# Julian-Wyatt/AnoDDPM

Measured on AMD Instinct MI355X. Metric: reverse-diffusion images/sec @256x256 T=1000 simplex, higher is better.
Workload: dtype f32; 1 GPU; 256x256 simplex(8 oct) T=1000 base128 attn16,8 batch4/GPU (BASELINE config 2); per_gpu_batch=4, global_batch=4, T=1000, parallelism=batch-sharded x1 (no data-path collective), output_finite=True

## Files before the change

anoddpm_amd/csrc/pointwise.hip:

```cpp
#include "common.h"

namespace {

typedef float f32x4 __attribute__((ext_vector_type(4)));
typedef float f32x16 __attribute__((ext_vector_type(16)));

constexpr int PW_WAVES = 8;
constexpr int PW_NT = PW_WAVES * 64;

template <int NB, int KMAX, int DBG = 0>
__global__ __launch_bounds__(PW_NT) void pointwise_stream_kernel(const anoddpm_igemm_args a, const int tiles, const int tiles_per_image)
{
    constexpr int NBP = NB + 2;
    constexpr int NTN = NB / 32;
    __shared__ __attribute__((aligned(16))) f32x4 wl[(KMAX / 4) * NBP];
    const int tid = threadIdx.x, lane = tid & 63, wave = tid >> 6;
    const int p = lane & 31, h = lane >> 5;
    const int K = a.c0 + a.c1, N = a.N;
    const int n0 = blockIdx.y * NB;
    const int nchunks = K >> 5;

    {
        const f32x4 *__restrict__ wg = reinterpret_cast<const f32x4 *>(a.bmat);
        const int total = (K >> 2) * NB;
        for (int idx = tid; idx < total; idx += PW_NT) {
            const int q = idx / NB, n = idx - q * NB;
            wl[q * NBP + n] = wg[(int64_t)q * N + n0 + n];
        }
    }
    __syncthreads();

    const int gw = blockIdx.x * PW_WAVES + wave, stride = gridDim.x * PW_WAVES;
    if (gw >= tiles) return;
    const int my_tiles = (tiles - gw + stride - 1) / stride;

    f32x4 ring[4][4];
    int ld_tile = 0, ld_chunk = 0;
    const float *ld_base0 = nullptr, *ld_base1 = nullptr;
    auto set_tile = [&](int t) {
        const int tile = gw + (t < my_tiles ? t : my_tiles - 1) * stride;
        const int b = tile / tiles_per_image, pl = (tile - b * tiles_per_image) * 32 + p;
        ld_base0 = a.a0 + (int64_t)b * a.a0_bs + (int64_t)pl * a.a0_ld + h * 16;
        ld_base1 = a.c1 ? a.a1 + (int64_t)b * a.a1_bs + (int64_t)pl * a.a1_ld + h * 16 : ld_base0;
    };
    auto issue = [&](f32x4 (&dst)[4]) {
        if ((DBG & 2) && ld_tile + ld_chunk > 2) return;
        const int c = ld_chunk * 32;
        const float *src = c < a.c0 ? ld_base0 + c : ld_base1 + (c - a.c0);
#pragma unroll
        for (int i = 0; i < 4; ++i) dst[i] = *reinterpret_cast<const f32x4 *>(src + 4 * i);
        if (++ld_chunk == nchunks) { ld_chunk = 0; set_tile(++ld_tile); }
    };
    set_tile(0);
    issue(ring[0]);
    issue(ring[1]);
    issue(ring[2]);
    if (wave >= PW_WAVES / 2 && my_tiles >= 2 && !(DBG & 4)) {
        for (int i = 0; i < nchunks / 2; ++i) __builtin_amdgcn_s_sleep(127);
    }

    const f32x4 *wrow = wl + h * 4 * NBP + p;
    f32x4 bq[2][NTN];
#pragma unroll
    for (int nt = 0; nt < NTN; ++nt) bq[0][nt] = wrow[nt * 32];
    for (int t = 0; t < my_tiles; ++t) {
        f32x16 acc[NTN];
#pragma unroll
        for (int nt = 0; nt < NTN; ++nt)
#pragma unroll
            for (int r = 0; r < 16; ++r) acc[nt][r] = 0.f;
        for (int j0 = 0; j0 < nchunks; j0 += 4) {
#pragma unroll
            for (int s = 0; s < 4; ++s) {
                issue(ring[(s + 3) & 3]);
                const int j = j0 + s;
                const f32x4 *wq = wrow + j * 8 * NBP;
                const f32x4 *wn = wrow + (j + 1 == nchunks ? 0 : j + 1) * 8 * NBP;
#pragma unroll
                for (int i = 0; i < 4; ++i) {
                    const f32x4 *nx = i < 3 ? wq + (i + 1) * NBP : wn;
#pragma unroll
                    for (int nt = 0; nt < NTN; ++nt) bq[(i + 1) & 1][nt] = nx[nt * 32];
                    __builtin_amdgcn_sched_barrier(0);
#pragma unroll
                    for (int e = 0; e < 4; ++e)
#pragma unroll
                        for (int nt = 0; nt < NTN; ++nt)
                            acc[nt] = __builtin_amdgcn_mfma_f32_32x32x2f32(bq[i & 1][nt][e], ring[s][i][e], acc[nt], 0, 0, 0);
                    __builtin_amdgcn_sched_barrier(0);
                }
            }
        }
        const int tile = gw + t * stride;
        const int b = tile / tiles_per_image, pl = (tile - b * tiles_per_image) * 32 + p;
        float *__restrict__ O = a.out + (int64_t)b * a.o_bs + (int64_t)pl * a.out_ld + n0 + 4 * h;
        const float *R = a.res ? a.res + (int64_t)b * a.r_bs + (int64_t)pl * a.res_ld + n0 + 4 * h : nullptr;
        const float *TE = a.temb ? a.temb + (int64_t)b * a.temb_ld + n0 + 4 * h : nullptr;
        const float *BI = a.bias ? a.bias + n0 + 4 * h : nullptr;
#pragma unroll
        for (int nt = 0; nt < NTN; ++nt) {
            f32x4 rv[4], add[4];
#pragma unroll
            for (int g = 0; g < 4; ++g) {
                const int c = nt * 32 + g * 8;
                rv[g] = R ? *reinterpret_cast<const f32x4 *>(R + c) : f32x4{0.f, 0.f, 0.f, 0.f};
                add[g] = BI ? *reinterpret_cast<const f32x4 *>(BI + c) : f32x4{0.f, 0.f, 0.f, 0.f};
                if (TE) add[g] += *reinterpret_cast<const f32x4 *>(TE + c);
            }
#pragma unroll
            for (int g = 0; g < 4; ++g) {
                f32x4 v;
#pragma unroll
                for (int e = 0; e < 4; ++e) v[e] = a.alpha * acc[nt][g * 4 + e] + add[g][e] + rv[g][e];
                if (!(DBG & 1) || v[0] == 12345.678f) *reinterpret_cast<f32x4 *>(O + nt * 32 + g * 8) = v;
            }
        }
    }
}

}

namespace anoddpm {

int launch_pointwise_stream(const anoddpm_igemm_args *a, hipStream_t s)
{
    const int K = a->c0 + a->c1;
    const int64_t P = (int64_t)a->H * a->W;
    ANODDPM_REQUIRE(a->ks == 1 && a->a_mode == 0 && a->b_mode == 0 && a->heads == 1 && a->ksplit == 1,
                    "pointwise stream: needs an unsplit 1x1 convolution with packed weights");
    ANODDPM_REQUIRE(!a->gn_scale && a->act == 0 && !a->stats, "pointwise stream: no fused GroupNorm / activation / statistics");
    ANODDPM_REQUIRE(K % 128 == 0 && a->c0 % 32 == 0 && K <= 512, "pointwise stream: K must be a multiple of 128, <= 512, sources split at a multiple of 32");
    ANODDPM_REQUIRE(P % 32 == 0 && a->N % 64 == 0, "pointwise stream: H*W must be a multiple of 32 and N of 64");
    const int64_t tiles = a->B * (P / 32);
    ANODDPM_REQUIRE(tiles < ((int64_t)1 << 31), "pointwise stream: too many pixels");
    const bool wide = (a->N % 128 == 0) && K <= 256;
    const int NB = wide ? 128 : 64;
    const int ny = a->N / NB;
    int gx = 256 / ny;
    const int64_t need = (tiles + PW_WAVES - 1) / PW_WAVES;
    if (gx > need) gx = (int)need;
    if (gx < 1) gx = 1;
    const dim3 grid((unsigned)gx, (unsigned)ny);
#ifdef ANODDPM_ABLATE
    const int dbg = anoddpm::g_debug[3];
#endif
    const int tpi = (int)(P / 32);
#define PW_LAUNCH(NB_, KMAX_, DBG_) \
    hipLaunchKernelGGL((pointwise_stream_kernel<NB_, KMAX_, DBG_>), grid, dim3(PW_NT), 0, s, *a, (int)tiles, tpi)
#ifdef ANODDPM_ABLATE
    if (wide && dbg == 1) PW_LAUNCH(128, 256, 1);
    else if (wide && dbg == 2) PW_LAUNCH(128, 256, 2);
    else if (wide && dbg == 3) PW_LAUNCH(128, 256, 3);
    else if (wide && dbg == 4) PW_LAUNCH(128, 256, 4);
    else
#endif
    if (wide) PW_LAUNCH(128, 256, 0);
    else PW_LAUNCH(64, 512, 0);
#undef PW_LAUNCH
    return check_launch("igemm(pointwise stream)");
}

}
```

anoddpm_amd/csrc/smallmap.hip:

```cpp
#include "common.h"

using anoddpm::silu_f;

namespace {

typedef float f32x4 __attribute__((ext_vector_type(4)));

constexpr int SM_NT = 512;

__host__ __device__ constexpr int sm_kch(int ks) { return ks == 3 ? 256 : 512; }
__host__ __device__ constexpr int sm_hpix(int ks, int tm, int w) { return ks == 1 ? tm : (tm / w + 2) * (w + 2); }

__device__ __forceinline__ __amdgpu_buffer_rsrc_t sm_rsrc(const float *base)
{
    return __builtin_amdgcn_make_buffer_rsrc(const_cast<float *>(base), 0, 0x7ffffffe, 0x00020000);
}
__device__ __forceinline__ f32x4 sm_bld4(__amdgpu_buffer_rsrc_t r, unsigned lane_bytes, unsigned wave_bytes)
{
    return __builtin_bit_cast(f32x4, __builtin_amdgcn_raw_buffer_load_b128(r, (int)lane_bytes, (int)wave_bytes, 0));
}

template <int KS, int RT, int CT, int LOG2W>
__global__ __launch_bounds__(SM_NT) void smallmap_kernel(const anoddpm_igemm_args a)
{
// ... 127 lines not shown
                    for (int u = 0; u < 4; ++u)
                        if (r0 + u < rows) { s += (double)v[u].x; qq += (double)v[u].y; }
                }
            }
            csum[2 * c] = s; csum[2 * c + 1] = qq;
        }
        __syncthreads();
        if (tid < groups) {
            double S = 0.0, Q = 0.0;
            for (int c = tid * cpg; c < (tid + 1) * cpg; ++c) { S += csum[2 * c]; Q += csum[2 * c + 1]; }
            const double n = (double)P * cpg;
            const double mean = S / n;
            double var = Q / n - mean * mean;
            var = var > 0.0 ? var : 0.0;
            gst[2 * tid] = mean;
            gst[2 * tid + 1] = 1.0 / sqrt(var + (double)a.fold_eps);
        }
        __syncthreads();
        for (int c = tid; c < Kpad; c += SM_NT) {
            float scv = 0.f, shv = 0.f;
            if (c < K) {
                const int g = c / cpg;
                const double sc = gst[2 * g + 1] * (double)a.fold_gamma[c];
                scv = (float)sc;
                shv = (float)((double)a.fold_beta[c] - gst[2 * g] * sc);
            }
            aff_sc[c] = scv; aff_sh[c] = shv;
        }
        __syncthreads();
    } else if (a.gn_scale) {
        for (int c = tid; c < Kpad; c += SM_NT) {
            aff_sc[c] = c < K ? a.gn_scale[(int64_t)b * a.gn_ld + c] : 0.f;
            aff_sh[c] = c < K ? a.gn_shift[(int64_t)b * a.gn_ld + c] : 0.f;
        }
        __syncthreads();
    }
    store_A(0);
    __syncthreads();

    int hp0[RT];
#pragma unroll
    for (int rt = 0; rt < RT; ++rt) {
        const int m = rt * 16 + l16;
        hp0[rt] = (KS == 1 ? m : (m >> LOG2W) * HP + (m & (W - 1))) * PITCH + 4 * q;
    }
    f32x4 acc[RT][CT];
#pragma unroll
    for (int rt = 0; rt < RT; ++rt)
#pragma unroll
        for (int ct = 0; ct < CT; ++ct) acc[rt][ct] = f32x4{0.f, 0.f, 0.f, 0.f};

    for (int chunk = 0; chunk < nchunks; ++chunk) {
        const float *Ab = Abuf + (chunk & (nbuf - 1)) * (HPIX * PITCH) + wave * CPW;
        const bool more = chunk + 1 < nchunks;
        if (more) load_A(chunk + 1);
        f32x4 av[2][RT];
        auto read_frags = [&](int s, int set) {
            const int tap = s / SPT, i = s % SPT;
            const int toff = (KS == 1 ? 0 : (tap / 3) * HP + (tap % 3)) * PITCH + 16 * i;
#pragma unroll
            for (int rt = 0; rt < RT; ++rt) av[set][rt] = *reinterpret_cast<const f32x4 *>(Ab + hp0[rt] + toff);
        };
        read_frags(0, 0);
#pragma unroll
        for (int s = 0; s < SPC; ++s) {
            const int cur = s & 1, slot = s % PD;
            if (s + 1 < SPC) read_frags(s + 1, cur ^ 1);
#pragma unroll
            for (int e = 0; e < 4; ++e)
#pragma unroll
                for (int rt = 0; rt < RT; ++rt)
#pragma unroll
                    for (int ct = 0; ct < CT; ++ct)
                        acc[rt][ct] = __builtin_amdgcn_mfma_f32_16x16x4f32(av[cur][rt][e], ring[slot][ct][e], acc[rt][ct], 0, 0, 0);
            const unsigned o = (s + PD < SPC) ? b_off(chunk, s + PD) : b_off(chunk + 1, s + PD - SPC);
#pragma unroll
            for (int ct = 0; ct < CT; ++ct) ring[slot][ct] = sm_bld4(rW, ulane, o + ct * 256u);
            __builtin_amdgcn_sched_barrier(0);
        }
        if (more) {
            if (nbuf == 1) __syncthreads();
            store_A(chunk + 1);
        }
        __syncthreads();
    }

    auto red_at = [&](int slot, int rt, int ct, int e) { return red + ((slot * TM + rt * 16 + 4 * q + e) * RP + ct * 16 + l16); };
    if (wave >= 4) {
#pragma unroll
        for (int rt = 0; rt < RT; ++rt)
#pragma unroll
            for (int ct = 0; ct < CT; ++ct)
#pragma unroll
                for (int e = 0; e < 4; ++e) *red_at(wave - 4, rt, ct, e) = acc[rt][ct][e];
    }
    __syncthreads();
    if (wave < 4) {
#pragma unroll
        for (int rt = 0; rt < RT; ++rt)
#pragma unroll
            for (int ct = 0; ct < CT; ++ct)
#pragma unroll
                for (int e = 0; e < 4; ++e) acc[rt][ct][e] += *red_at(wave, rt, ct, e);
    }
    __syncthreads();
    if (wave < 4) {
#pragma unroll
        for (int rt = 0; rt < RT; ++rt)
#pragma unroll
            for (int ct = 0; ct < CT; ++ct)
#pragma unroll
                for (int e = 0; e < 4; ++e) *red_at(wave, rt, ct, e) = acc[rt][ct][e];
    }
    __syncthreads();
    float *O = a.out + (int64_t)b * a.o_bs;
    const float *R = a.res ? a.res + (int64_t)b * a.r_bs : nullptr;
    const float *TE = a.temb ? a.temb + (int64_t)b * a.temb_ld : nullptr;
    constexpr int ITEMS = TM * (TN / 4);
    for (int it = tid; it < ITEMS; it += SM_NT) {
        const int row = it / (TN / 4), c4 = it - row * (TN / 4);
        const float *r0 = red + row * RP + c4 * 4;
        f32x4 v = *reinterpret_cast<const f32x4 *>(r0);
        v += *reinterpret_cast<const f32x4 *>(r0 + TM * RP);
        v += *reinterpret_cast<const f32x4 *>(r0 + 2 * TM * RP);
        v += *reinterpret_cast<const f32x4 *>(r0 + 3 * TM * RP);
        const int n = n0 + c4 * 4;
        v = v * a.alpha;
        if (a.bias) v += *reinterpret_cast<const f32x4 *>(a.bias + n);
        if (TE) v += *reinterpret_cast<const f32x4 *>(TE + n);
        if (R) v += *reinterpret_cast<const f32x4 *>(R + (int64_t)(p0 + row) * a.res_ld + n);
        *reinterpret_cast<f32x4 *>(O + (int64_t)(p0 + row) * a.out_ld + n) = v;
        if (a.stats) *reinterpret_cast<f32x4 *>(red + (4 * TM + row) * RP + c4 * 4) = v;
    }
    if (a.stats) {
        __syncthreads();
        if (tid < TN) {
            const float *col = red + 4 * TM * RP + tid;
            float s = 0.f, qq = 0.f;
#pragma unroll 4
            for (int r = 0; r < TM; ++r) { const float v = col[r * RP]; s += v; qq += v * v; }
            float *st = a.stats + (((int64_t)b * (P / TM) + p0 / TM) * N + n0 + tid) * 2;
            st[0] = s; st[1] = qq;
        }
    }
}

}

namespace anoddpm {

int smallmap_tile(int ks, int H, int W, int K, int c0, int N, int B)
{
    const int P = H * W;
    if (!(ks == 1 || ks == 3) || P > 256 || P < 16 || (W != 4 && W != 8 && W != 16) || H * W != P) return 0;
    if (K % 16 || c0 % 4 || K > 1024 || N % 32 || K < 16) return 0;
    const int M = B * P;
    static const int cand[4][2] = {{2, 6}, {1, 6}, {2, 2}, {1, 2}};
    int best = 0;
    for (int c = 0; c < 4; ++c) {
        const int rt = cand[c][0], ct = cand[c][1];
        const int tm = 16 * rt, tn = 16 * ct;
        if (P % tm || tm % W || N % tn) continue;
        if (ks == 3 && ct == 6) continue;
        const int wgs = (M / tm) * (N / tn);
        if (wgs >= 200) return rt * 16 + ct;
        best = rt * 16 + ct;
    }
    return best;
}

int launch_smallmap(const anoddpm_igemm_args *a, hipStream_t s)
{
    const int K = a->c0 + a->c1;
    ANODDPM_REQUIRE(a->b_mode == 0 && a->heads == 1 && a->a_mode == 0 && a->ksplit == 1, "smallmap: needs packed weights, heads 1, a_mode 0, ksplit 1");
    const int tile = smallmap_tile(a->ks, a->H, a->W, K, a->c0, a->N, a->B);
    ANODDPM_REQUIRE(tile != 0, "smallmap: shape not supported (H*W <= 256, W in {4, 8, 16}, K %% 16 == 0, 16 <= K <= 1024, N %% 32 == 0)");
    ANODDPM_REQUIRE(a->c1 == 0 || a->a1, "smallmap: dual source needs a1");
    ANODDPM_REQUIRE(a->out_ld % 4 == 0 && (!a->res || a->res_ld % 4 == 0) && a->a0_ld % 4 == 0 && (a->c1 == 0 || a->a1_ld % 4 == 0),
                    "smallmap: pixel strides must be multiples of 4 floats");
    ANODDPM_REQUIRE(!a->tail_csum, "smallmap: no split-K tail");
    ANODDPM_REQUIRE(!a->gn_scale || a->gn_shift, "smallmap: gn_scale without gn_shift");
    if (a->fold_gamma) {
        ANODDPM_REQUIRE(a->fold_beta && a->fold_stats0 && (a->c1 == 0 || a->fold_stats1), "smallmap: GroupNorm fold: null pointer");
        ANODDPM_REQUIRE(a->fold_groups >= 1 && a->fold_groups <= 64 && K % a->fold_groups == 0, "smallmap: GroupNorm fold: bad group count");
        ANODDPM_REQUIRE((a->fold_fmt0 != 0 || a->fold_rows0 >= 1) && (a->c1 == 0 || a->fold_fmt1 != 0 || a->fold_rows1 >= 1),
                        "smallmap: GroupNorm fold: statistics rows missing");
    }
    const int rt = tile >> 4, ct = tile & 15;
    const int TM = 16 * rt, TN = 16 * ct;
    const int P = a->H * a->W;
    const int kch = sm_kch(a->ks);
    const int nchunks = (K + kch - 1) / kch, Kpad = nchunks * kch;
    const int hpix = sm_hpix(a->ks, TM, a->W);
    size_t stage = (size_t)(nchunks > 1 ? 2 : 1) * hpix * (kch + 4) * sizeof(float);
    const size_t fold = (size_t)(2 * Kpad + 128) * sizeof(double);
    const size_t redb = (size_t)5 * TM * (TN + 4) * sizeof(float);
    if (stage < fold) stage = fold;
    if (stage < redb) stage = redb;
    const size_t lds = (size_t)2 * Kpad * sizeof(float) + stage;
    ANODDPM_REQUIRE(lds <= 160 * 1024, "smallmap: LDS budget exceeded");
    dim3 grid((unsigned)(a->N / TN), (unsigned)((int64_t)a->B * P / TM));
#define SM_LAUNCH(KS_, RT_, CT_, LW_)                                                                                     \
    do {                                                                                                                  \
        static bool attr_done[ANODDPM_MAX_DEV];                                                                           \
        if (int rc_ = allow_big_lds(reinterpret_cast<const void *>(&smallmap_kernel<KS_, RT_, CT_, LW_>), attr_done,      \
                                    "igemm(smallmap)"))                                                                   \
            return rc_;                                                                                                   \
        hipLaunchKernelGGL((smallmap_kernel<KS_, RT_, CT_, LW_>), grid, dim3(SM_NT), lds, s, *a);                         \
        return check_launch("igemm(smallmap)");                                                                           \
    } while (0)
    const int lw = a->W == 4 ? 2 : (a->W == 8 ? 3 : 4);
    if (a->ks == 3) {
        if (rt == 1 && ct == 2) { if (lw == 2) SM_LAUNCH(3, 1, 2, 2); if (lw == 3) SM_LAUNCH(3, 1, 2, 3); SM_LAUNCH(3, 1, 2, 4); }
        if (rt == 2 && ct == 2) { if (lw == 2) SM_LAUNCH(3, 2, 2, 2); if (lw == 3) SM_LAUNCH(3, 2, 2, 3); SM_LAUNCH(3, 2, 2, 4); }
    } else {
        if (rt == 1 && ct == 2) SM_LAUNCH(1, 1, 2, 3);
        if (rt == 1 && ct == 6) SM_LAUNCH(1, 1, 6, 3);
        if (rt == 2 && ct == 2) SM_LAUNCH(1, 2, 2, 3);
        if (rt == 2 && ct == 6) SM_LAUNCH(1, 2, 6, 3);
    }
#undef SM_LAUNCH
    set_error("smallmap: no instantiation for tile %d x %d", TM, TN);
    return ANODDPM_EINVAL;
}

}

extern "C" int anoddpm_smallmap_tile(int32_t ks, int32_t H, int32_t W, int32_t K, int32_t c0, int32_t N, int32_t B)
{
    return anoddpm::smallmap_tile(ks, H, W, K, c0, N, B);
}
```

anoddpm_amd/unet.py:

```python
import ctypes
import math
import os
from types import SimpleNamespace

import numpy as np
import torch
from torch import nn

from . import _lib
from ._lib import (AttentionArgs, ChanStatsArgs, GnFinalizeArgs, HeadArgs, IgemmArgs, LayoutArgs, LinearArgs, Op, PackArgs, PackBatchArgs,
                   PosembArgs, ResampleArgs, SoftmaxArgs, StemArgs, check, lib)

__all__ = ["UNetModel", "update_ema_params", "zero_module", "GroupNorm32"]

_DEFAULT_MULTS = {512: (0.5, 1, 1, 2, 2, 4, 4), 256: (1, 1, 2, 2, 4, 4), 128: (1, 1, 2, 3, 4),
                  64: (1, 2, 3, 4), 32: (1, 2, 3, 4)}


class _Affine(nn.Module):

    def __init__(self, c):
        super().__init__()
        self.weight = nn.Parameter(torch.ones(c))
        self.bias = nn.Parameter(torch.zeros(c))
# ... 156 lines not shown
                return _indexed(conv=_Weights((cout, cin, 3, 3))) if blk[4] == "conv" else nn.Module()
            heads = n_heads if n_head_channels == -1 else None
            if heads is None:
                assert cin % n_head_channels == 0, \
                    f"q,k,v channels {cin} is not divisible by num_head_channels {n_head_channels}"
            return _AttentionParams(cin)

        def seq(blks):
            d = nn.ModuleDict()
            for b in blks:
                d[b[0].split(".")[-1]] = make(b)
            return d

        self.down = nn.ModuleList([seq(b) for b in down])
        self.middle = seq(middle)
        self.up = nn.ModuleList([seq(b) for b in up])
        self.out = _indexed(_0=_Affine(out_ch), _2=_Weights((in_channels, self._final_cin, 3, 3), zero=True))
        self._plans = {}
        self._tplans = {}
        self._weights_epoch = 0

    def mark_weights_changed(self):
        self._weights_epoch += 1

    def _heads_for(self, c):
        return self.num_heads if self.num_head_channels == -1 else c // self.num_head_channels

    def __deepcopy__(self, memo):
        import copy
        cls = self.__class__
        new = cls.__new__(cls)
        memo[id(self)] = new
        for k, v in self.__dict__.items():
            if k in ("_plans", "_tplans"):
                new.__dict__[k] = {}
            else:
                new.__dict__[k] = copy.deepcopy(v, memo)
        return new

    def __getstate__(self):
        d = dict(self.__dict__)
        d["_plans"] = {}
        d["_tplans"] = {}
        return d

    def forward(self, x, time):
        needs_grad = torch.is_grad_enabled() and (x.requires_grad or any(p.requires_grad for p in self.parameters()))
        if needs_grad:
            return self._forward_autograd(x, time)
        if self.training and self.dropout > 0:
            return self._forward_train_mode_no_grad(x, time)
        return self.forward_hip(x, time)

    def _forward_train_mode_no_grad(self, x, time):
        _lib.require_cuda(x, "UNetModel.forward (train mode)")
        if not (x.dim() == 4 and x.shape[2] == x.shape[3] and x.shape[1] == self.in_channels):
            raise ValueError(f"expected [B,{self.in_channels},S,S] input, got {tuple(x.shape)}")
        from . import train_plan
        B, S = x.shape[0], x.shape[2]
        if not train_plan.eligible(self, B, S):
            raise NotImplementedError(f"UNetModel in train() mode with dropout at batch {B}, size {S}: outside the native training plan; "
                                      "call .eval() for sampling")
        plan = self._train_plan_for(B, S, x.device, False, float(self.dropout))
        xin = x.detach()
        if xin.dtype != torch.float32 or not xin.is_contiguous():
            xin = xin.float().contiguous()
        if xin.data_ptr() % 16:
            xin = xin.clone()
        t = time.detach()
        if t.dtype != torch.int64 or t.device != x.device or not t.is_contiguous():
            t = t.to(device=x.device, dtype=torch.int64).contiguous()
        y = plan.run_forward(xin, t)
        plan.fwd_epoch = getattr(plan, "fwd_epoch", 0) + 1
        return y.clone().to(x.dtype)

    def forward_hip(self, x, time, out=None, borrow=False):
        _lib.require_cuda(x, "UNetModel.forward")
        B, C, H, W = x.shape
        if C != self.in_channels or H != W:
            raise ValueError(f"expected [B,{self.in_channels},S,S] input, got {tuple(x.shape)}")
        plan = self._plan_for(B, H, x.device)
        xin = x.detach()
        if xin.dtype != torch.float32 or not xin.is_contiguous():
            xin = xin.float().contiguous()
        if xin.data_ptr() % 16:
            xin = xin.clone()
        t = time.detach()
        if t.dtype != torch.int64 or t.device != x.device or not t.is_contiguous():
            t = t.to(device=x.device, dtype=torch.int64).contiguous()
        y = plan.run(xin, t)
        if out is not None:
            out.copy_(y.view_as(out))
            return out
        if borrow and x.dtype == torch.float32:
            return y.view_as(x)
        return y.clone().to(x.dtype)

    def _plan_for(self, B, S, device):
        key = (B, S, device, os.environ.get("ANODDPM_ARITH", "fp32"))
        plan = self._plans.get(key)
        if plan is None:
            plan = _Plan(self, B, S, device)
            self._plans[key] = plan
        plan.refresh_weights()
        return plan

    def _train_plan_for(self, B, S, device, want_dx, p_drop=0.0):
        from .train_plan import TrainPlan
        key = (B, S, device, bool(want_dx), float(p_drop))
        plan = self._tplans.get(key)
        if plan is None or not plan.params_match():
            plan = self._tplans[key] = TrainPlan(self, B, S, device, want_dx=want_dx, p_drop=p_drop)
        return plan

    def _forward_autograd(self, x, time):
        _lib.require_cuda(x, "UNetModel.forward (training)")
        if not (x.dim() == 4 and x.shape[2] == x.shape[3] and x.shape[1] == self.in_channels):
            raise ValueError(f"expected [B,{self.in_channels},S,S] input, got {tuple(x.shape)}")
        from . import train_plan
        from .training import reducer_of
        B, S = x.shape[0], x.shape[2]
        if not train_plan.eligible(self, B, S):
            raise NotImplementedError(f"UNetModel training at batch {B}, size {S}, base {self.model_channels}: outside the native "
                                      "training plan (1 <= batch <= 16 per GPU, base_channels % 4 == 0 and <= 256, <= 4 image channels)")
        red = reducer_of(self)
        if red is not None:
            red.flat.bind_grads()
        p_drop = float(self.dropout) if (self.training and self.dropout > 0) else 0.0
        plan = self._train_plan_for(B, S, x.device, x.requires_grad, p_drop)
        anchor = next((p for p in self.parameters() if p.requires_grad), x)
        return train_plan.TrainPlanFunction.apply(x, time, anchor, plan)


def _posemb_freqs(half):
    step = np.log(10000) / half
    return torch.exp(torch.arange(half) * -step)


class _GnFold:
    """A GroupNorm that is finished inside its consumer (anoddpm_igemm_args.fold_*): statistics sources (pointer, rows, format)
    of the one or two concatenated tensors + the affine parameters."""


def _use_winograd():
    import os
    return os.environ.get("ANODDPM_NO_WINOGRAD", "0") != "1"


def fused_attention_ok(L, ch):
    return (L % 16 == 0 and 16 <= L <= 1024 and 16 <= ch <= 512 and (ch & (ch - 1)) == 0
            and os.environ.get("ANODDPM_NO_FUSED_ATTENTION", "0") != "1")


def smallmap_ok(H, W, K, N, B, *, ks, a_mode=0, b_mode=0, heads=1, c0=None):
    if os.environ.get("ANODDPM_NO_SMALLMAP", "0") == "1" or a_mode != 0 or b_mode != 0 or heads != 1:
        return False
    P = H * W
    if ks == 3 and P > int(os.environ.get("ANODDPM_SMALLMAP_CONV_MAXP", 64)) and P * B > int(os.environ.get("ANODDPM_SMALLMAP_CONV_MAXM", 256)):
        return False
    if ks == 1 and P > int(os.environ.get("ANODDPM_SMALLMAP_GEMM_MAXP", 256)):
        return False
    return lib().anoddpm_smallmap_tile(ks, H, W, K, K if c0 is None else c0, N, B) != 0


def wino23s_ok(H, W, K, N, B, *, ks, a_mode=0, b_mode=0, heads=1, c0=None):
    if os.environ.get("ANODDPM_NO_WINO23S", "0") == "1" or ks != 3 or b_mode != 0 or heads != 1 or not _use_winograd():
        return False
    if K > int(os.environ.get("ANODDPM_WINO23S_MAXK", 256)):
        return False
    return lib().anoddpm_wino23s_tile(H, W, K, K if c0 is None else c0, N, B, a_mode) != 0


F43_MAX_GN_K = 1024


def choose_conv_cfg(H, W, K, N, Z, *, ks=3, a_mode=0, b_mode=0, heads=1, c0=None, c1=0, wino=True, f43=False, plain=False, small=False):
    c0 = K if c0 is None else c0
    P = H * W
    if small and smallmap_ok(H, W, K, N, Z, ks=ks, a_mode=a_mode, b_mode=b_mode, heads=heads, c0=c0):
        return 5, 1
    if small and wino and wino23s_ok(H, W, K, N, Z, ks=ks, a_mode=a_mode, b_mode=b_mode, heads=heads, c0=c0):
        return 6, 1
    if (plain and ks == 1 and a_mode == 0 and b_mode == 0 and heads == 1 and K % 128 == 0 and K <= 512 and c0 % 32 == 0
            and P % 32 == 0 and N % 64 == 0 and os.environ.get("ANODDPM_NO_STREAM1X1", "0") != "1"):
        nb = 128 if (N % 128 == 0 and K <= 256) else 64
        if (Z * P // 32) * (N // nb) >= int(os.environ.get("ANODDPM_STREAM1X1_MIN_TILES", 1024)):
            return 4, 1

    def ok128():
        if P % 128:
            return False
        if ks == 1:
            return True
        tw = min(W, 32)
        th = 128 // tw
        return th <= H and H % th == 0
    blocks128 = (P // 128) * ((N + 127) // 128) * Z if ok128() else 0
    cfg = 0 if (blocks128 >= 256 and N >= 96) else 1
    wino_blocks = (H // 16) * (W // 16) * ((N + 63) // 64) * Z
    wino_ksplit = 1
    wino_ok = (wino and ks == 3 and b_mode == 0 and heads == 1 and a_mode in (0, 1) and H % 16 == 0 and W % 16 == 0
               and K % 16 == 0 and (c1 == 0 or c0 % 16 == 0) and N >= 32 and _use_winograd())
    if wino_ok and wino_blocks < 200:
        wch = K // 16
        wino_ksplit = int(min(max(1, wch // 4), -(-256 // wino_blocks)))
        if N % 4 or wino_blocks * wino_ksplit < 128 or os.environ.get("ANODDPM_NO_WINOGRAD_SPLITK"):
            wino_ok = False
        else:
            cps = -(-wch // wino_ksplit)
            wino_ksplit = -(-wch // cps)
    f43 = f43 and (plain or K <= F43_MAX_GN_K)
    if (wino_ok and f43 and N % 128 == 0 and H * W == 32 * 32 and K >= int(os.environ.get("ANODDPM_F43_32_MINK", 512))
            and os.environ.get("ANODDPM_F43_32", "1") == "1"):
        wg = (H // 16) * (W // 16) * (N // 128) * Z
        ks43 = int(min(max(1, (K // 16) // 4), -(-256 // wg)))
        cps = -(-(K // 16) // ks43)
        ks43 = -(-(K // 16) // cps)
        if wg * ks43 >= 200:
            return 3, ks43
    if wino_ok and f43 and N % 64 == 0 and H * W >= int(os.environ.get("ANODDPM_F43_MIN_PIXELS", 64 * 64)) \
            and (H // 16) * (W // 16) * (N // 64) * Z >= 128 and os.environ.get("ANODDPM_NO_F43", "0") != "1":
        wg128 = (H // 16) * (W // 16) * (N // 128) * Z if N % 128 == 0 else 0
        if 100 <= wg128 < 200 and K // 16 >= 8 and os.environ.get("ANODDPM_F43_SPLITK", "0") == "1":
            return 3, 2
        if 0 < wg128 <= 64 and os.environ.get("ANODDPM_F43_DEEP_SPLITK", "1") == "1":
            ks43 = int(min(max(1, (K // 16) // 4), -(-256 // wg128)))
            cps = -(-(K // 16) // ks43)
            ks43 = -(-(K // 16) // cps)
            if ks43 > 1 and wg128 * ks43 >= 200:
                return 3, ks43
        return 3, 1
    if wino_ok:
        return 2, wino_ksplit
    bm = 128 if cfg == 0 else 64
    blocks = -(-P // bm) * ((N + bm - 1) // bm) * Z
    nchunks = (K + 31) // 32
    ksplit = 1
    target = int(os.environ.get("ANODDPM_SPLITK_TARGET", 512))
    if blocks < target and nchunks > 1 and N % 4 == 0:
        ksplit = int(min(nchunks, 16, max(1, -(-target // blocks))))
    return cfg, ksplit


PACK_KINDS = {"conv3": 0, "wino": 1, "conv1": 2, "small": 3, "copy": 4, "wino43": 5}
_PACK_TAPS = {0: 9, 1: 16, 2: 1, 3: 9, 4: 1, 5: 36}


def pack_kind(kind, shape):
    if kind == "conv":
        kind = "conv3" if (len(shape) == 4 and shape[2] == 3) else "conv1"
    return PACK_KINDS[kind]


def pack_floats(kind, N, K, bwd=0, kc=0):
    return N * kc if (kind == PACK_KINDS["conv1"] and bwd) else _PACK_TAPS[kind] * N * K


def _op_array(ops):
    arr = (Op * len(ops))()
    for i, (code, st) in enumerate(ops):
        arr[i].code = code
        arr[i].flags = 0
        arr[i].args = ctypes.addressof(st)
    return arr


def _pack_table(jobs, device):
    arr = (PackArgs * len(jobs))()
    block0 = [0]
    for i, st in enumerate(jobs):
        ctypes.memmove(ctypes.addressof(arr[i]), ctypes.addressof(st), ctypes.sizeof(PackArgs))
        block0.append(block0[-1] + int(lib().anoddpm_pack_job_blocks(ctypes.byref(st))))
    raw = torch.frombuffer(bytearray(bytes(arr)), dtype=torch.uint8).to(device)
    b0 = torch.tensor(block0, dtype=torch.int32).to(device)
    pb = PackBatchArgs()
    pb.jobs, pb.block0, pb.njobs, pb.nblocks = raw.data_ptr(), b0.data_ptr(), len(jobs), block0[-1]
    return pb, raw, b0


class _Plan:
    honours_arith = True
    honours_csum = True

    def __init__(self, model, B, S, device):
        self.model = model
        self.B, self.S, self.device = B, S, device
        self.keep = []
        self.ops = []
        self._pack_jobs = []
        self._bf16_jobs = []
        self._packed = {}
        self.arith = os.environ.get("ANODDPM_ARITH", "fp32") if self.honours_arith else "fp32"
        if self.arith not in ("fp32", "bf16split3"):
            raise ValueError(f"ANODDPM_ARITH={self.arith}: expected fp32 or bf16split3")
        self.token = None
        self.igemm_flops = 0.0
        self._ws_need = 0
        self.stats_of = {}
        self.igemm_log = []
        self.block_out = {}
        self.csum_mode = self.honours_csum and os.environ.get("ANODDPM_CSUM", "0") == "1"
        self._csum_arena, self._csum_used = None, 0
        if self.csum_mode:
            cap = 2 * B * sum(p.shape[0] for p in model.parameters() if p.dim() == 4 and p.shape[-1] == 3)
            self._csum_arena = torch.zeros(max(cap, 2), dtype=torch.float64, device=device)
            self.keep.append(self._csum_arena)
        with torch.no_grad():
            self._build()
        if self.csum_mode and getattr(self, "posemb", None) is not None:
            self.posemb.zero = self._csum_arena.data_ptr() if self._csum_used else None
            self.posemb.zero_doubles = self._csum_used
        self.op_array = _op_array(self.ops)

    def buf(self, *shape, dtype=torch.float32):
        t = torch.empty(*shape, dtype=dtype, device=self.device)
        self.keep.append(t)
        return t

    def packed(self, key, kind, out=None):
        ck = (key, kind, None if out is None else out.data_ptr())
        hit = self._packed.get(ck)
        if hit is not None:
            return hit
        p = dict(self.model.named_parameters())[key]
        shape = tuple(p.shape)
        if kind == "wino43b":
            N, K = shape[0], shape[1]
            dst = torch.empty(54 * N * K, dtype=torch.float32, device=self.device)
            self.keep.append(dst)
            self._bf16_jobs.append((key, dst, N, K))
            self._packed[ck] = dst
            return dst
        k = pack_kind(kind, shape)
        N, K = (p.numel(), 1) if k == PACK_KINDS["copy"] else (shape[0], shape[1])
        n_out = pack_floats(k, N, K)
        if k not in (PACK_KINDS["small"], PACK_KINDS["copy"]) and K % 4:
            raise NotImplementedError(f"{key}: input channel count {K} must be a multiple of 4")
        dst = out if out is not None else torch.empty(n_out, dtype=torch.float32, device=self.device)
        self.keep.append(dst)
        st = PackArgs()
# ... 544 lines not shown
```

Before: 0.4507 images/s.

## Overlap weight staging and epilogue loads in pointwise 1x1 stream kernel

The pointwise 1x1 stream kernel now issues its first activation loads before staging weights into LDS, and batches the weight copy eight loads deep. It precomputes the bias plus timestep-embedding row per wave in dynamic LDS, prefetches residual values during the last K chunk group, and specialises on the presence of a residual. The host falls back to the narrower N tile when the wide tile would underfill the grid, and the smallmap kernel is extended to plain 32x32 1x1 convolutions. The change adds dynamic-LDS attribute setup and overlap checks, and it shifts kernel choice for mid-size maps, which could pick a slower path on some shapes.

```diff
diff --git a/anoddpm_amd/csrc/pointwise.hip b/anoddpm_amd/csrc/pointwise.hip
--- a/anoddpm_amd/csrc/pointwise.hip
+++ b/anoddpm_amd/csrc/pointwise.hip
@@ -8,31 +8,20 @@
 constexpr int PW_WAVES = 8;
 constexpr int PW_NT = PW_WAVES * 64;
 
-template <int NB, int KMAX, int DBG = 0>
+template <int NB, bool RES, int DBG = 0>
 __global__ __launch_bounds__(PW_NT) void pointwise_stream_kernel(const anoddpm_igemm_args a, const int tiles, const int tiles_per_image)
 {
     constexpr int NBP = NB + 2;
     constexpr int NTN = NB / 32;
-    __shared__ __attribute__((aligned(16))) f32x4 wl[(KMAX / 4) * NBP];
-    const int tid = threadIdx.x, lane = tid & 63, wave = tid >> 6;
+    extern __shared__ __attribute__((aligned(16))) f32x4 wl[];
+    const int tid = threadIdx.x, lane = tid & 63;
+    const int wave = __builtin_amdgcn_readfirstlane(tid >> 6);
     const int p = lane & 31, h = lane >> 5;
     const int K = a.c0 + a.c1, N = a.N;
     const int n0 = blockIdx.y * NB;
     const int nchunks = K >> 5;
-
-    {
-        const f32x4 *__restrict__ wg = reinterpret_cast<const f32x4 *>(a.bmat);
-        const int total = (K >> 2) * NB;
-        for (int idx = tid; idx < total; idx += PW_NT) {
-            const int q = idx / NB, n = idx - q * NB;
-            wl[q * NBP + n] = wg[(int64_t)q * N + n0 + n];
-        }
-    }
-    __syncthreads();
-
     const int gw = blockIdx.x * PW_WAVES + wave, stride = gridDim.x * PW_WAVES;
-    if (gw >= tiles) return;
-    const int my_tiles = (tiles - gw + stride - 1) / stride;
+    const int my_tiles = gw < tiles ? (tiles - gw + stride - 1) / stride : 0;
 
     f32x4 ring[4][4];
     int ld_tile = 0, ld_chunk = 0;
@@ -51,10 +40,52 @@
         for (int i = 0; i < 4; ++i) dst[i] = *reinterpret_cast<const f32x4 *>(src + 4 * i);
         if (++ld_chunk == nchunks) { ld_chunk = 0; set_tile(++ld_tile); }
     };
-    set_tile(0);
-    issue(ring[0]);
-    issue(ring[1]);
-    issue(ring[2]);
+    f32x4 *addrow = wl + (K >> 2) * NBP + wave * (NB / 4);
+    f32x4 bt = {0.f, 0.f, 0.f, 0.f}, tt = {0.f, 0.f, 0.f, 0.f};
+    auto add_request = [&](int t) {
+        const int tile = gw + (t < my_tiles ? t : my_tiles - 1) * stride;
+        const int b = tile / tiles_per_image, ql = lane & (NB / 4 - 1);
+        bt = *reinterpret_cast<const f32x4 *>(a.bias ? a.bias + n0 + 4 * ql : a.bmat);
+        tt = *reinterpret_cast<const f32x4 *>(a.temb ? a.temb + (int64_t)b * a.temb_ld + n0 + 4 * ql : a.bmat);
+    };
+    auto add_write = [&]() {
+        f32x4 add = a.bias ? bt : f32x4{0.f, 0.f, 0.f, 0.f};
+        if (a.temb) add += tt;
+        addrow[lane & (NB / 4 - 1)] = add;
+        __builtin_amdgcn_wave_barrier();
+    };
+    if (my_tiles > 0) {
+        set_tile(0);
+        issue(ring[0]);
+        issue(ring[1]);
+        issue(ring[2]);
+        add_request(0);
+    }
+    __builtin_amdgcn_sched_barrier(0);
+
+    {
+        const f32x4 *__restrict__ wg = reinterpret_cast<const f32x4 *>(a.bmat);
+        const int total = (K >> 2) * NB;
+        for (int idx0 = tid; idx0 < total; idx0 += 8 * PW_NT) {
+            f32x4 v[8];
+#pragma unroll
+            for (int u = 0; u < 8; ++u) {
+                const int idx = idx0 + u * PW_NT < total ? idx0 + u * PW_NT : idx0;
+                const int q = idx / NB, n = idx - q * NB;
+                v[u] = wg[(int64_t)q * N + n0 + n];
+            }
+#pragma unroll
+            for (int u = 0; u < 8; ++u) {
+                const int idx = idx0 + u * PW_NT;
+                const int q = idx / NB, n = idx - q * NB;
+                if (idx < total) wl[q * NBP + n] = v[u];
+            }
+        }
+    }
+    __syncthreads();
+    if (my_tiles <= 0) return;
+    add_write();
+
     if (wave >= PW_WAVES / 2 && my_tiles >= 2 && !(DBG & 4)) {
         for (int i = 0; i < nchunks / 2; ++i) __builtin_amdgcn_s_sleep(127);
     }
@@ -63,59 +94,84 @@
     f32x4 bq[2][NTN];
 #pragma unroll
     for (int nt = 0; nt < NTN; ++nt) bq[0][nt] = wrow[nt * 32];
-    for (int t = 0; t < my_tiles; ++t) {
-        f32x16 acc[NTN];
+    f32x16 acc[NTN];
+    float *O = nullptr;
+    const float *R = nullptr;
+    f32x4 rv[NTN][4];
+    auto ep_request = [&](int nt, int slot) __attribute__((always_inline)) {
+        if (!RES) return;
+#pragma unroll
+        for (int g = 0; g < 4; ++g) rv[slot][g] = *reinterpret_cast<const f32x4 *>(R + nt * 32 + g * 8);
+    };
+    const f32x4 *addq = addrow + h;
+    auto ep_store = [&](int nt, int slot) __attribute__((always_inline)) {
+#pragma unroll
+        for (int g = 0; g < 4; ++g) {
+            const f32x4 add = addq[nt * 8 + g * 2];
+            const f32x4 r = RES ? rv[slot][g] : f32x4{0.f, 0.f, 0.f, 0.f};
+            f32x4 v;
+#pragma unroll
+            for (int e = 0; e < 4; ++e) v[e] = a.alpha * acc[nt][g * 4 + e] + add[e] + r[e];
+            if (!(DBG & 1) || v[0] == 12345.678f) *reinterpret_cast<f32x4 *>(O + nt * 32 + g * 8) = v;
+        }
+    };
+    auto chunk_group = [&](int j0, bool tail) __attribute__((always_inline)) {
+#pragma unroll
+        for (int s = 0; s < 4; ++s) {
+            if (!tail || s == 0) issue(ring[(s + 3) & 3]);
+            const int j = j0 + s;
+            const f32x4 *wq = wrow + j * 8 * NBP;
+            const f32x4 *wn = wrow + (j + 1 == nchunks ? 0 : j + 1) * 8 * NBP;
+#pragma unroll
+            for (int i = 0; i < 4; ++i) {
+                const f32x4 *nx = i < 3 ? wq + (i + 1) * NBP : wn;
+#pragma unroll
+                for (int nt = 0; nt < NTN; ++nt) bq[(i + 1) & 1][nt] = nx[nt * 32];
+                __builtin_amdgcn_sched_barrier(0);
+#pragma unroll
+                for (int e = 0; e < 4; ++e)
+#pragma unroll
+                    for (int nt = 0; nt < NTN; ++nt)
+                        acc[nt] = __builtin_amdgcn_mfma_f32_32x32x2f32(bq[i & 1][nt][e], ring[s][i][e], acc[nt], 0, 0, 0);
+                __builtin_amdgcn_sched_barrier(0);
+            }
+            if (tail && s + 1 < NTN) {
+                ep_request(s + 1, s + 1);
+                __builtin_amdgcn_sched_barrier(0);
+            }
+        }
+    };
+    auto tile_body = [&](int t, bool last) __attribute__((always_inline)) {
 #pragma unroll
         for (int nt = 0; nt < NTN; ++nt)
 #pragma unroll
             for (int r = 0; r < 16; ++r) acc[nt][r] = 0.f;
-        for (int j0 = 0; j0 < nchunks; j0 += 4) {
-#pragma unroll
-            for (int s = 0; s < 4; ++s) {
-                issue(ring[(s + 3) & 3]);
-                const int j = j0 + s;
-                const f32x4 *wq = wrow + j * 8 * NBP;
-                const f32x4 *wn = wrow + (j + 1 == nchunks ? 0 : j + 1) * 8 * NBP;
-#pragma unroll
-                for (int i = 0; i < 4; ++i) {
-                    const f32x4 *nx = i < 3 ? wq + (i + 1) * NBP : wn;
-#pragma unroll
-                    for (int nt = 0; nt < NTN; ++nt) bq[(i + 1) & 1][nt] = nx[nt * 32];
-                    __builtin_amdgcn_sched_barrier(0);
-#pragma unroll
-                    for (int e = 0; e < 4; ++e)
-#pragma unroll
-                        for (int nt = 0; nt < NTN; ++nt)
-                            acc[nt] = __builtin_amdgcn_mfma_f32_32x32x2f32(bq[i & 1][nt][e], ring[s][i][e], acc[nt], 0, 0, 0);
-                    __builtin_amdgcn_sched_barrier(0);
-                }
-            }
-        }
-        const int tile = gw + t * stride;
-        const int b = tile / tiles_per_image, pl = (tile - b * tiles_per_image) * 32 + p;
-        float *__restrict__ O = a.out + (int64_t)b * a.o_bs + (int64_t)pl * a.out_ld + n0 + 4 * h;
-        const float *R = a.res ? a.res + (int64_t)b * a.r_bs + (int64_t)pl * a.res_ld + n0 + 4 * h : nullptr;
-        const float *TE = a.temb ? a.temb + (int64_t)b * a.temb_ld + n0 + 4 * h : nullptr;
-        const float *BI = a.bias ? a.bias + n0 + 4 * h : nullptr;
-#pragma unroll
-        for (int nt = 0; nt < NTN; ++nt) {
-            f32x4 rv[4], add[4];
-#pragma unroll
-            for (int g = 0; g < 4; ++g) {
-                const int c = nt * 32 + g * 8;
-                rv[g] = R ? *reinterpret_cast<const f32x4 *>(R + c) : f32x4{0.f, 0.f, 0.f, 0.f};
-                add[g] = BI ? *reinterpret_cast<const f32x4 *>(BI + c) : f32x4{0.f, 0.f, 0.f, 0.f};
-                if (TE) add[g] += *reinterpret_cast<const f32x4 *>(TE + c);
-            }
-#pragma unroll
-            for (int g = 0; g < 4; ++g) {
-                f32x4 v;
-#pragma unroll
-                for (int e = 0; e < 4; ++e) v[e] = a.alpha * acc[nt][g * 4 + e] + add[g][e] + rv[g][e];
-                if (!(DBG & 1) || v[0] == 12345.678f) *reinterpret_cast<f32x4 *>(O + nt * 32 + g * 8) = v;
-            }
-        }
-    }
+        {
+            const int tile = gw + t * stride;
+            const int b = tile / tiles_per_image, pl = (tile - b * tiles_per_image) * 32 + p;
+            O = a.out + (int64_t)b * a.o_bs + (int64_t)pl * a.out_ld + n0 + 4 * h;
+            if (RES) R = a.res + (int64_t)b * a.r_bs + (int64_t)pl * a.res_ld + n0 + 4 * h;
+        }
+        if (last) {
+            for (int j0 = 0; j0 + 4 < nchunks; j0 += 4) chunk_group(j0, false);
+            ep_request(0, 0);
+            __builtin_amdgcn_sched_barrier(0);
+            chunk_group(nchunks - 4, true);
+#pragma unroll
+            for (int nt = 0; nt < NTN; ++nt) ep_store(nt, nt);
+        } else {
+            for (int j0 = 0; j0 < nchunks; j0 += 4) chunk_group(j0, false);
+            add_request(t + 1);
+#pragma unroll
+            for (int nt = 0; nt < NTN; ++nt) {
+                ep_request(nt, 0);
+                ep_store(nt, 0);
+            }
+            add_write();
+        }
+    };
+    for (int t = 0; t + 1 < my_tiles; ++t) tile_body(t, false);
+    tile_body(my_tiles - 1, true);
 }
 
 }
@@ -133,7 +189,18 @@
     ANODDPM_REQUIRE(P % 32 == 0 && a->N % 64 == 0, "pointwise stream: H*W must be a multiple of 32 and N of 64");
     const int64_t tiles = a->B * (P / 32);
     ANODDPM_REQUIRE(tiles < ((int64_t)1 << 31), "pointwise stream: too many pixels");
-    const bool wide = (a->N % 128 == 0) && K <= 256;
+    if (a->res && a->res != a->out) {
+        const float *re = a->res + (int64_t)a->B * a->r_bs, *oe = a->out + (int64_t)a->B * a->o_bs;
+        ANODDPM_REQUIRE(re <= a->out || oe <= a->res, "pointwise stream: the residual overlaps the output without being the output");
+    } else if (a->res) {
+        ANODDPM_REQUIRE(a->res_ld == a->out_ld && a->r_bs == a->o_bs, "pointwise stream: an in-place residual needs the output's strides");
+    }
+    bool wide = (a->N % 128 == 0) && K <= 256;
+    if (wide) {
+        const int64_t need128 = (tiles + PW_WAVES - 1) / PW_WAVES;
+        const int64_t gx128 = need128 < 256 / (a->N / 128) ? need128 : 256 / (a->N / 128);
+        if (gx128 * (a->N / 128) < 256 && tiles * (a->N / 64) >= 2048) wide = false;
+    }
     const int NB = wide ? 128 : 64;
     const int ny = a->N / NB;
     int gx = 256 / ny;
@@ -141,22 +208,35 @@
     if (gx > need) gx = (int)need;
     if (gx < 1) gx = 1;
     const dim3 grid((unsigned)gx, (unsigned)ny);
+    const size_t lds = ((size_t)(K / 4) * (NB + 2) + (size_t)PW_WAVES * (NB / 4)) * sizeof(f32x4);
 #ifdef ANODDPM_ABLATE
     const int dbg = anoddpm::g_debug[3];
 #endif
     const int tpi = (int)(P / 32);
-#define PW_LAUNCH(NB_, KMAX_, DBG_) \
-    hipLaunchKernelGGL((pointwise_stream_kernel<NB_, KMAX_, DBG_>), grid, dim3(PW_NT), 0, s, *a, (int)tiles, tpi)
+#define PW_LAUNCH1(NB_, RES_, DBG_)                                                                                        \
+    do {                                                                                                                   \
+        static bool attr_done[ANODDPM_MAX_DEV];                                                                            \
+        if (int rc_ = allow_big_lds(reinterpret_cast<const void *>(&pointwise_stream_kernel<NB_, RES_, DBG_>), attr_done,  \
+                                    "igemm(pointwise stream)"))                                                            \
+            return rc_;                                                                                                    \
+        hipLaunchKernelGGL((pointwise_stream_kernel<NB_, RES_, DBG_>), grid, dim3(PW_NT), lds, s, *a, (int)tiles, tpi);    \
+    } while (0)
+#define PW_LAUNCH(NB_, DBG_)                                                                                               \
+    do {                                                                                                                   \
+        if (a->res) PW_LAUNCH1(NB_, true, DBG_);                                                                           \
+        else PW_LAUNCH1(NB_, false, DBG_);                                                                                 \
+    } while (0)
 #ifdef ANODDPM_ABLATE
-    if (wide && dbg == 1) PW_LAUNCH(128, 256, 1);
-    else if (wide && dbg == 2) PW_LAUNCH(128, 256, 2);
-    else if (wide && dbg == 3) PW_LAUNCH(128, 256, 3);
-    else if (wide && dbg == 4) PW_LAUNCH(128, 256, 4);
+    if (wide && dbg == 1) PW_LAUNCH(128, 1);
+    else if (wide && dbg == 2) PW_LAUNCH(128, 2);
+    else if (wide && dbg == 3) PW_LAUNCH(128, 3);
+    else if (wide && dbg == 4) PW_LAUNCH(128, 4);
     else
 #endif
-    if (wide) PW_LAUNCH(128, 256, 0);
-    else PW_LAUNCH(64, 512, 0);
+    if (wide) PW_LAUNCH(128, 0);
+    else PW_LAUNCH(64, 0);
 #undef PW_LAUNCH
+#undef PW_LAUNCH1
     return check_launch("igemm(pointwise stream)");
 }
 
diff --git a/anoddpm_amd/csrc/smallmap.hip b/anoddpm_amd/csrc/smallmap.hip
--- a/anoddpm_amd/csrc/smallmap.hip
+++ b/anoddpm_amd/csrc/smallmap.hip
@@ -303,7 +303,8 @@
 int smallmap_tile(int ks, int H, int W, int K, int c0, int N, int B)
 {
     const int P = H * W;
-    if (!(ks == 1 || ks == 3) || P > 256 || P < 16 || (W != 4 && W != 8 && W != 16) || H * W != P) return 0;
+    const bool w_ok = W == 4 || W == 8 || W == 16 || (ks == 1 && W == 32);
+    if (!(ks == 1 || ks == 3) || P > (ks == 1 ? 1024 : 256) || P < 16 || !w_ok) return 0;
     if (K % 16 || c0 % 4 || K > 1024 || N % 32 || K < 16) return 0;
     const int M = B * P;
     static const int cand[4][2] = {{2, 6}, {1, 6}, {2, 2}, {1, 2}};
@@ -311,7 +312,7 @@
     for (int c = 0; c < 4; ++c) {
         const int rt = cand[c][0], ct = cand[c][1];
         const int tm = 16 * rt, tn = 16 * ct;
-        if (P % tm || tm % W || N % tn) continue;
+        if (P % tm || (ks == 3 && tm % W) || N % tn) continue;
         if (ks == 3 && ct == 6) continue;
         const int wgs = (M / tm) * (N / tn);
         if (wgs >= 200) return rt * 16 + ct;
@@ -325,7 +326,7 @@
     const int K = a->c0 + a->c1;
     ANODDPM_REQUIRE(a->b_mode == 0 && a->heads == 1 && a->a_mode == 0 && a->ksplit == 1, "smallmap: needs packed weights, heads 1, a_mode 0, ksplit 1");
     const int tile = smallmap_tile(a->ks, a->H, a->W, K, a->c0, a->N, a->B);
-    ANODDPM_REQUIRE(tile != 0, "smallmap: shape not supported (H*W <= 256, W in {4, 8, 16}, K %% 16 == 0, 16 <= K <= 1024, N %% 32 == 0)");
+    ANODDPM_REQUIRE(tile != 0, "smallmap: shape not supported (H*W <= 256 and W in {4, 8, 16}, 1x1 also 32x32; K %% 16 == 0, 16 <= K <= 1024, N %% 32 == 0)");
     ANODDPM_REQUIRE(a->c1 == 0 || a->a1, "smallmap: dual source needs a1");
     ANODDPM_REQUIRE(a->out_ld % 4 == 0 && (!a->res || a->res_ld % 4 == 0) && a->a0_ld % 4 == 0 && (a->c1 == 0 || a->a1_ld % 4 == 0),
                     "smallmap: pixel strides must be multiples of 4 floats");
diff --git a/anoddpm_amd/unet.py b/anoddpm_amd/unet.py
--- a/anoddpm_amd/unet.py
+++ b/anoddpm_amd/unet.py
@@ -332,10 +332,12 @@
             and os.environ.get("ANODDPM_NO_FUSED_ATTENTION", "0") != "1")
 
 
-def smallmap_ok(H, W, K, N, B, *, ks, a_mode=0, b_mode=0, heads=1, c0=None):
+def smallmap_ok(H, W, K, N, B, *, ks, a_mode=0, b_mode=0, heads=1, c0=None, skip1x1=False):
     if os.environ.get("ANODDPM_NO_SMALLMAP", "0") == "1" or a_mode != 0 or b_mode != 0 or heads != 1:
         return False
     P = H * W
+    if skip1x1:
+        return ks == 1 and 256 < P <= 1024 and K <= 512 and lib().anoddpm_smallmap_tile(ks, H, W, K, K if c0 is None else c0, N, B) != 0
     if ks == 3 and P > int(os.environ.get("ANODDPM_SMALLMAP_CONV_MAXP", 64)) and P * B > int(os.environ.get("ANODDPM_SMALLMAP_CONV_MAXM", 256)):
         return False
     if ks == 1 and P > int(os.environ.get("ANODDPM_SMALLMAP_GEMM_MAXP", 256)):
@@ -364,8 +366,13 @@
     if (plain and ks == 1 and a_mode == 0 and b_mode == 0 and heads == 1 and K % 128 == 0 and K <= 512 and c0 % 32 == 0
             and P % 32 == 0 and N % 64 == 0 and os.environ.get("ANODDPM_NO_STREAM1X1", "0") != "1"):
         nb = 128 if (N % 128 == 0 and K <= 256) else 64
-        if (Z * P // 32) * (N // nb) >= int(os.environ.get("ANODDPM_STREAM1X1_MIN_TILES", 1024)):
+        tiles = Z * P // 32
+        if nb == 128 and min(256 // (N // 128), -(-tiles // 8)) * (N // 128) < 256 and tiles * (N // 64) >= 2048:
+            nb = 64
+        if tiles * (N // nb) >= int(os.environ.get("ANODDPM_STREAM1X1_MIN_TILES", 1024)):
             return 4, 1
+    if small and plain and smallmap_ok(H, W, K, N, Z, ks=ks, a_mode=a_mode, b_mode=b_mode, heads=heads, c0=c0, skip1x1=True):
+        return 5, 1
 
     def ok128():
         if P % 128:
```

New measurement: 0.4534 images/s, median of 6. About the same (+0.6%).
